# CircleRadon/TokenPacker

Hardware: NVIDIA H100
Metric: compressed_visual_tokens_per_sec (higher is better)
Workload: dtype bf16

## Files before the change

### tokenpacker_b200/csrc/tp_api.cu

```cuda
#include <limits.h>
#include <atomic>
#include <math.h>
#include <stdio.h>
#include <stdlib.h>
#include <string.h>
#include <map>
#include <tuple>
#include <vector>

#include "../../include/tokenpacker_b200.h"
#include "../../include/tokenpacker_b200_clip_tower.h"
#include "../../include/tokenpacker_b200_clip_tower_f16.h"
#include "../../include/tokenpacker_b200_clip_tower_train.h"
#include "../../include/tokenpacker_b200_clip_tower_ckpt.h"
#include "../../include/tokenpacker_b200_clip_tower_embed.h"
#include "../../include/tokenpacker_b200_clip_u8.h"
#include "../../include/tokenpacker_b200_hd_u8.h"
#include "../../include/tokenpacker_b200_input_grad.h"
#include "../../include/tokenpacker_b200_layers.h"
#include "../../include/tokenpacker_b200_jpeg.h"
#include "tp_gemm.cuh"
#include "tp_kernels.cuh"
#include "tp_backward.cuh"
#include "tp_clip_tower.cuh"
// ... 205 lines not shown
template <int kBlockN, bool kTower, bool kF16 = false>
int launch_gemm_tt(const GemmItem& it, const CUtensorMap& map_a, const CUtensorMap& map_b, int sms, cudaStream_t stream) {
  using Cfg = GemmConfig<kBlockN>;
  {
    static thread_local unsigned attr_done = 0;
    int dev = 0;
    TP_CUDA(cudaGetDevice(&dev));
    if (dev >= 32 || !(attr_done & (1u << dev))) {
      TP_CUDA(cudaFuncSetAttribute(tp_gemm_kernel<kBlockN, kTower, kF16>, cudaFuncAttributeMaxDynamicSharedMemorySize, Cfg::kSmemBytes));
      if (dev < 32) attr_done |= 1u << dev;
    }
  }
  const long long tiles = ((it.M + kBlockM - 1) / kBlockM) * ((it.N + kBlockN - 1) / kBlockN);
  const int grid = static_cast<int>(tiles < sms ? tiles : sms);
  GemmEpilogue ep = it.ep;
  TP_CUDA(launch_pdl(tp_gemm_kernel<kBlockN, kTower, kF16>, dim3(grid), dim3(kGemmThreads), Cfg::kSmemBytes, stream, map_a, map_b,
                     static_cast<int>(it.M), static_cast<int>(it.N), static_cast<int>(it.K), static_cast<int>(it.a.seg_rows), ep));
  return TP_OK;
}

template <int kBlockN>
int launch_gemm_t(const GemmItem& it, const CUtensorMap& map_a, const CUtensorMap& map_b, int sms, cudaStream_t stream) {
  switch (gemm_variant(it.ep)) {
    case 2: return launch_gemm_tt<kBlockN, true, true>(it, map_a, map_b, sms, stream);
    case 1: return launch_gemm_tt<kBlockN, true>(it, map_a, map_b, sms, stream);
    default: return launch_gemm_tt<kBlockN, false>(it, map_a, map_b, sms, stream);
  }
}

struct BuiltLaunch {
  GemmGroup g;
  PeerStores peers;
  int grid;
};

int build_pair_group(const GemmItem* items, int count, int sms, const FrontWork* front, BuiltLaunch* out) {
  using Cfg = Gemm2Config;
  GemmGroup& g = out->g;
  memset(&g, 0, sizeof(g));
  g.count = count;
  for (int i = 1; i < count; ++i)
    if (gemm_variant(items[i].ep) != gemm_variant(items[0].ep)) return TP_ERR_INVALID_ARGUMENT;
  if (count > 0 && gemm_variant(items[0].ep) != 0 && front != nullptr) return TP_ERR_INVALID_ARGUMENT;
  long long total = 0;
  for (int i = 0; i < count; ++i) {
    const GemmItem& it = items[i];
    GemmProblem& p = g.p[i];
    if (it.kind == 1) {
      if (it.N != kC || it.K != kC || it.a2 == nullptr || it.b2 == nullptr || (it.attn.s != 2 && it.attn.s != 4)) return TP_ERR_INVALID_ARGUMENT;
      TP_TRY(make_map_2d(&p.tmap_a, it.a.ptr, it.M, it.K, it.a.ld, kBlockM));
      TP_TRY(make_map_2d(&p.tmap_a2, it.a2, it.M, it.K, it.a.ld, kBlockM));
      TP_TRY(make_map_2d(&p.tmap_b, it.b, it.N, it.K, it.ldb, Cfg::kTileN / 2));
      TP_TRY(make_map_2d(&p.tmap_b2, it.b2, it.N, it.K, it.ldb, Cfg::kTileN / 2));
      p.kind = 1;
      p.attn = it.attn;
      p.a_parts = 1;
      p.M = static_cast<int>(it.M);
      p.N = static_cast<int>(it.N);
      p.K = static_cast<int>(it.K);
      p.num_n_blocks = 4;
      p.num_k_blocks = static_cast<int>(it.K / kBlockK);
      p.tiles_mn = static_cast<int>((it.M + Cfg::kTileM - 1) / Cfg::kTileM) * p.num_n_blocks;
      p.k_splits = 1;
      p.kb_per_split = p.num_k_blocks;
      p.num_tiles = p.tiles_mn;
      p.dep_counter = nullptr;
      total += p.num_tiles;
      continue;
    }
    if (it.tn == 1 && (it.b_parts > 1 || it.b_seg_rows != 0)) {
      if (it.b_parts < 1 || it.b_parts > kMaxAParts || it.N % (it.b_parts * Cfg::kTileN) != 0 || it.a.parts > 1 || it.a.seg_rows != 0 ||
          (it.b_seg_rows != 0 && (it.b_seg_rows % kBlockK != 0 || it.K % it.b_seg_rows != 0)))
        return TP_ERR_INVALID_ARGUMENT;
      TP_TRY(make_map_2d(&p.tmap_a, it.a.ptr, it.K, it.M, it.a.ld, 64));
      const long long np = it.N / it.b_parts;
      for (int q = 0; q < it.b_parts; ++q) {
// ... 51 lines not shown
        int rows = p.c_unit << lvl;
        if (rows > kBlockM || rows > it.ep.seg_len) rows = p.c_unit;
        TP_TRY(make_map_3d(lvl == 0 ? &p.tmap_c : &p.tmap_cx[lvl - 1], it.ep.c, it.M / it.ep.seg_len, it.ep.seg_len, it.N, it.ep.ldc,
                           it.ep.seg_stride * it.ep.ldc, rows));
      }
    } else {
      TP_TRY(make_map_2d(&p.tmap_c, it.ep.c, it.M, it.N, it.ep.ldc, kBlockM));
    }
    if (it.ep.dual) {
      if (!p.use_tma_store || c_segmented || it.ep.wm_s != 0 || it.n_peers > 0 || !it.ep.gelu || it.c_pre == nullptr || it.k_splits > 1)
        return TP_ERR_INVALID_ARGUMENT;
      TP_TRY(make_map_2d(&p.tmap_cx[0], it.c_pre, it.M, it.N, it.ld_pre, kBlockM));
    }
    p.M = static_cast<int>(it.M);
    p.N = static_cast<int>(it.N);
    p.K = static_cast<int>(it.K);
    p.a_seg_rows = static_cast<int>(it.a.seg_rows);
    p.num_n_blocks = static_cast<int>((it.N + Cfg::kTileN - 1) / Cfg::kTileN);
    p.num_k_blocks = static_cast<int>((it.K + kBlockK - 1) / kBlockK);
    p.tiles_mn = static_cast<int>((it.M + Cfg::kTileM - 1) / Cfg::kTileM) * p.num_n_blocks;
    p.k_splits = it.k_splits;
    p.kb_per_split = (p.num_k_blocks + p.k_splits - 1) / p.k_splits;
    if (static_cast<long long>(p.k_splits - 1) * p.kb_per_split >= p.num_k_blocks) return TP_ERR_INVALID_ARGUMENT;
    p.c_split_stride = it.M * it.ep.ldc;
    p.num_tiles = p.tiles_mn * p.k_splits;
    p.ep = it.ep;
    p.done_counter = it.done_counter;
    p.dep_counter = it.dep_counter;
    p.dep_target = it.dep_target;
    p.dep_shift = it.dep_shift;
    p.dep_span = it.dep_span;
    p.dep_src_blocks = it.dep_src_blocks;
    p.dep_per = it.dep_per;
    if ((p.done_counter != nullptr && !p.use_tma_store) || (p.dep_counter != nullptr && (it.tn || it.a.seg_rows != 0)))
      return TP_ERR_INVALID_ARGUMENT;
    p.peer_out = it.n_peers > 0 ? 1 : 0;
    total += p.num_tiles;
  }
  if (total > 0x7fffffffll) return TP_ERR_INVALID_ARGUMENT;
  g.total_tiles = static_cast<int>(total);
  if (front != nullptr) g.front = *front;
  PeerStores& peers = out->peers;
  memset(&peers, 0, sizeof(peers));
  int peer_item = -1;
  for (int i = 0; i < count; ++i)
    if (items[i].n_peers > 0 || g.p[i].c_seg_len != 0) {
      if (peer_item >= 0 && items[i].n_peers == 0 && items[peer_item].n_peers == 0 && g.p[i].c_seg_len > kBlockM) continue;
      if (peer_item >= 0) return TP_ERR_INVALID_ARGUMENT;
      peer_item = i;
    }
  if (peer_item >= 0) {
    const GemmItem& it0 = items[peer_item];
    const GemmProblem& p0 = g.p[peer_item];
    void* const local_dst[1] = {it0.ep.c};
    void* const* dst = it0.n_peers > 0 ? it0.peer_c : local_dst;
    const int n_dst = it0.n_peers > 0 ? it0.n_peers : 1;
    if (n_dst > kMaxPeers || it0.ep.seg_row_offset != nullptr) return TP_ERR_INVALID_ARGUMENT;
    const bool whole = p0.c_seg_len != 0 && p0.c_seg_len <= kBlockM;
    if (p0.c_seg_len != 0) {
      int worst = 0;
      for (int a0 = 0; a0 > -p0.c_seg_len; a0 -= p0.c_unit) {
        int pieces = 0, a = a0;
        while (a < kBlockM) {
          if (whole && a >= 0 && a + p0.c_seg_len <= kBlockM) {
            int k = 1;
            while (k < kWholeLevels && a + (k + 1) * p0.c_seg_len <= kBlockM) ++k;
            ++pieces;
// ... 11 lines not shown
    }
    for (int p = 0; p < n_dst; ++p) {
      if (p0.c_seg_len != 0) {
        const long long n_segs = it0.M / it0.ep.seg_len;
        for (int lvl = 0; lvl < kBoxLevels; ++lvl) {
          int rows = p0.c_unit << lvl;
          if (rows > kBlockM || rows > it0.ep.seg_len) rows = p0.c_unit;
          TP_TRY(make_map_3d(&peers.m[p][lvl], dst[p], n_segs, it0.ep.seg_len, it0.N, it0.ep.ldc, it0.ep.seg_stride * it0.ep.ldc, rows));
        }
        for (int k = 1; k <= kWholeLevels; ++k) {
          const int kk = (whole && k * it0.ep.seg_len <= kBlockM && k <= n_segs) ? k : 1;
          if (whole)
            TP_TRY(make_map_3d(&peers.m[p][kBoxLevels + k - 1], dst[p], n_segs, it0.ep.seg_len, it0.N, it0.ep.ldc,
                               it0.ep.seg_stride * it0.ep.ldc, it0.ep.seg_len, kk));
          else
            peers.m[p][kBoxLevels + k - 1] = peers.m[p][0];
        }
      } else {
        TP_TRY(make_map_2d(&peers.m[p][0], dst[p], it0.M, it0.N, it0.ep.ldc, kBlockM));
      }
    }
    peers.count = n_dst;
    peers.whole = whole ? 1 : 0;
    g.p[peer_item].peer_out = 1;
  }
  const long long max_pairs = sms / 2;
  const int grid = 2 * static_cast<int>(total < max_pairs ? total : max_pairs);
  for (int i = 0; i < count; ++i)
    if (g.p[i].dep_shift == 31) g.p[i].dep_target = grid;
  out->grid = grid;
  return TP_OK;
}

template <bool kTower, bool kF16 = false>
int launch_built_t(const BuiltLaunch& b, cudaStream_t stream) {
  using Cfg = Gemm2Config;
  {
    static thread_local unsigned attr_done = 0;
    int dev = 0;
    TP_CUDA(cudaGetDevice(&dev));
    if (dev >= 32 || !(attr_done & (1u << dev))) {
      TP_CUDA(cudaFuncSetAttribute(tp_gemm2_kernel<kTower, kF16>, cudaFuncAttributeMaxDynamicSharedMemorySize, Cfg::kSmemBytes));
      if (dev < 32) attr_done |= 1u << dev;
    }
  }
  TP_CUDA(launch_pdl(tp_gemm2_kernel<kTower, kF16>, dim3(b.grid), dim3(kGemmThreads), Cfg::kSmemBytes, stream, b.g, b.peers));
  return TP_OK;
}

int launch_built(const BuiltLaunch& b, cudaStream_t stream) {
  int variant = 0;
  for (int i = 0; i < b.g.count; ++i) variant = gemm_variant(b.g.p[i].ep) > variant ? gemm_variant(b.g.p[i].ep) : variant;
  switch (variant) {
    case 2: return launch_built_t<true, true>(b, stream);
    case 1: return launch_built_t<true>(b, stream);
    default: return launch_built_t<false>(b, stream);
  }
}

int launch_gemm_pair_group(const GemmItem* items, int count, int sms, cudaStream_t stream, const FrontWork* front = nullptr,
                           BuiltLaunch* built = nullptr) {
  BuiltLaunch local;
  BuiltLaunch* b = built != nullptr ? built : &local;
  TP_TRY(build_pair_group(items, count, sms, front, b));
  return launch_built(*b, stream);
}

int choose_kernel(const GemmItem& it, int count, int sms, int mode) {
  const bool c_segmented = it.ep.seg_row_offset == nullptr && !it.ep.out_f32 && it.ep.seg_stride != 0 && it.ep.seg_stride != it.ep.seg_len;
  const bool pair_ok = (it.N % 256 == 0) && sms >= 2 && !(c_segmented && seg_store_unit(it.ep.seg_len) < 4);
  const bool pair_only = it.n_peers > 0 || it.tn || it.ep.dual || it.a.parts > 1 || it.k_splits > 1 || it.ep.out_f32 || it.kind == 1 || it.ep.wm_s != 0;
  if (pair_only && !pair_ok) return -1;
  const bool needs_256 = it.ep.stats_out != nullptr;
  const long long kb = (it.K + kBlockK - 1) / kBlockK;
  auto waves = [](long long tiles, long long units) { return (tiles + units - 1) / units; };
  const long long t_pair = ((it.M + 255) / 256) * ((it.N + 255) / 256);
  const long long t_256 = ((it.M + 127) / 128) * ((it.N + 255) / 256);
  const long long t_128 = ((it.M + 127) / 128) * ((it.N + 127) / 128);
  const long long c_pair = pair_ok ? waves(t_pair, sms / 2) * kb * 1024 * 9 / 8 : LLONG_MAX;
  const long long c_256 = (it.N % 256 == 0) ? waves(t_256, sms) * kb * 1024 : LLONG_MAX;
  const long long c_128 = needs_256 ? LLONG_MAX : waves(t_128, sms) * kb * 512 * 6 / 5;
  const long long launch = 10000;
  const long long l_pair = pair_ok ? c_pair + launch / count : LLONG_MAX;
  const long long l_256 = c_256 == LLONG_MAX ? LLONG_MAX : c_256 + launch;
  const long long l_128 = c_128 == LLONG_MAX ? LLONG_MAX : c_128 + launch;
  int choice;
  if (pair_only || mode == 2 || mode == 3) choice = 0;
  else if (mode == 1) choice = (it.N % 256 == 0) ? 1 : 2;
  else if (l_pair <= l_256 && l_pair <= l_128) choice = 0;
  else choice = (l_256 <= l_128) ? 1 : 2;
  if (choice == 0 && !pair_ok) choice = (it.N % 256 == 0) ? 1 : 2;
  return choice;
}

int gemm_mode() {
  const char* mode_env = getenv("TP_GEMM_MODE");
  return mode_env != nullptr ? atoi(mode_env) : 0;
}

int launch_gemms(const GemmItem* items, int count, int sms, cudaStream_t stream) {
  if (count <= 0 || count > kMaxGroup || mixed_precision(items, count)) return TP_ERR_INVALID_ARGUMENT;
  const int mode = gemm_mode();
  int choice[kMaxGroup];
  CUtensorMap map_a[kMaxGroup], map_b[kMaxGroup];
  GemmItem grouped[kMaxGroup];
  int n_grouped = 0;
  BuiltLaunch pair;
  for (int i = 0; i < count; ++i) {
    TP_TRY(check_item(items[i]));
    const GemmItem& it = items[i];
    if (it.n_peers > 0 && count != 1) return TP_ERR_INVALID_ARGUMENT;
    choice[i] = choose_kernel(it, count, sms, mode);
    if (choice[i] < 0) return TP_ERR_INVALID_ARGUMENT;
    if (choice[i] == 0) {
      if (mode == 3) TP_TRY(build_pair_group(&it, 1, sms, nullptr, &pair));
      else grouped[n_grouped++] = it;
    } else {
      TP_TRY(make_one_cta_maps(it, choice[i] == 1 ? 256 : 128, &map_a[i], &map_b[i]));
    }
  }
  if (n_grouped > 0) TP_TRY(build_pair_group(grouped, n_grouped, sms, nullptr, &pair));
  for (int i = 0; i < count; ++i) {
    if (choice[i] == 0) {
      if (mode == 3) TP_TRY(launch_gemm_pair_group(&items[i], 1, sms, stream));
    } else if (choice[i] == 1) {
      TP_TRY(launch_gemm_t<256>(items[i], map_a[i], map_b[i], sms, stream));
    } else {
      TP_TRY(launch_gemm_t<128>(items[i], map_a[i], map_b[i], sms, stream));
    }
  }
  if (n_grouped > 0) TP_TRY(launch_built(pair, stream));
  return TP_OK;
}

int launch_front_s(int s, const __nv_bfloat16* x0, long long x0_stride, __nv_bfloat16* q, long long Q, cudaStream_t stream);

bool chain_enabled(int mode) {
  const char* e = getenv("TP_CHAIN");
  const bool chain_off = e != nullptr && atoi(e) == 0;
  return !chain_off && (mode == 0 || mode == 2);
}

bool chain_feasible(const GemmItem* items, int count, int sms, bool by_cost = true) {
  const int mode = gemm_mode();
  if (!chain_enabled(mode) || count <= 0 || count > kMaxGroup || sms < 2) return false;
  for (int i = 0; i < count; ++i) {
    if (check_item(items[i]) != TP_OK || items[i].ep.seg_row_offset != nullptr || items[i].N % 256 != 0) return false;
    if (by_cost && choose_kernel(items[i], count, sms, mode) != 0) return false;
  }
  return true;
}

int launch_chain(GemmItem* items, int count, int* flags, long long flag_capacity, const FrontWork* front, int sms, cudaStream_t stream,
                 BuiltLaunch* built = nullptr) {
  if (count <= 0 || count > kMaxGroup || mixed_precision(items, count)) return TP_ERR_INVALID_ARGUMENT;
  for (int i = 0; i < count; ++i) {
    const int deps[3] = {items[i].dep, items[i].dep2, items[i].dep3};
    for (int d : deps) {
      if (d == kDepFront ? front == nullptr : (d >= 0 && (d >= i || items[d].stage >= items[i].stage))) return TP_ERR_INVALID_ARGUMENT;
      if (d >= 0 && items[i].kind == 0 && items[d].kind == 0 && (items[d].M != items[i].M || items[i].a.seg_rows != 0)) return TP_ERR_INVALID_ARGUMENT;
    }
  }
  bool fused_items = false;
  for (int i = 0; i < count; ++i) fused_items = fused_items || items[i].kind == 1 || items[i].ep.wm_s != 0;
  const bool chain = flags != nullptr && chain_feasible(items, count, sms, !fused_items);
  if (chain) {
    long long used = 0;
    FrontWork fw;
    memset(&fw, 0, sizeof(fw));
    if (front != nullptr) {
      if (used + 1 > flag_capacity) return TP_ERR_WORKSPACE_TOO_SMALL;
      fw = *front;
      fw.done_counter = flags + used;
      used += 1;
    }
    for (int i = 0; i < count; ++i) {
      bool produces = false;
      for (int j = 0; j < count; ++j) produces = produces || items[j].dep == i || items[j].dep2 == i || items[j].dep3 == i;
      if (!produces) continue;
      const long long out_rows = items[i].kind == 1 ? items[i].M / (items[i].attn.s * items[i].attn.s) : items[i].M;
      const long long blocks = (out_rows + 255) / 256;
      if (used + blocks > flag_capacity) return TP_ERR_WORKSPACE_TOO_SMALL;
      items[i].done_counter = flags + used;
      if (items[i].kind == 1) {
        items[i].attn.done_counter = items[i].done_counter;
        items[i].done_counter = nullptr;
      }
      used += blocks;
    }
    auto counter_of = [&](int d) { return items[d].kind == 1 ? items[d].attn.done_counter : items[d].done_counter; };
    auto gemm_target = [&](int d) { return 4 * static_cast<int>((items[d].N + 255) / 256); };
    for (int i = 0; i < count; ++i) {
      GemmItem& it = items[i];
      if (it.kind == 1) {
        if (it.dep < 0 || it.dep2 < 0 || it.dep3 < 0 || items[it.dep].M != it.M || items[it.dep2].M != it.M) return TP_ERR_INVALID_ARGUMENT;
        it.attn.k_counter = counter_of(it.dep);
        it.attn.v_counter = counter_of(it.dep2);
        it.attn.kv_target = gemm_target(it.dep);
        it.attn.q_counter = counter_of(it.dep3);
        it.attn.q_target = gemm_target(it.dep3);
        continue;
      }
      const int d = it.dep;
      if (d == kDepFront) {
        it.dep_counter = fw.done_counter;
        it.dep_shift = 31;
      } else if (d >= 0 && items[d].kind == 1) {
        it.dep_counter = counter_of(d);
        it.dep_span = items[d].attn.s * items[d].attn.s;
        it.dep_src_blocks = static_cast<int>((items[d].M + 255) / 256);
        it.dep_per = 8;
      } else if (d >= 0) {
        it.dep_counter = counter_of(d);
        it.dep_target = gemm_target(d);
      }
    }
    return launch_gemm_pair_group(items, count, sms, stream, front != nullptr ? &fw : nullptr, built);
  }
  for (int i = 0; i < count; ++i)
    if (items[i].kind == 1 || items[i].ep.wm_s != 0) return TP_ERR_INVALID_ARGUMENT;
  if (front != nullptr) TP_TRY(launch_front_s(front->s, front->x0, front->crop_stride, front->q, front->n_queries, stream));
  for (int first = 0; first < count;) {
    int last = first;
    while (last + 1 < count && items[last + 1].stage == items[first].stage) ++last;
    TP_TRY(launch_gemms(items + first, last - first + 1, sms, stream));
    first = last + 1;
  }
  return TP_OK;
}

int launch_gemm(const AOperand& a, const void* b, long long ldb, long long M, long long N, long long K, const GemmEpilogue& ep,
                int sms, cudaStream_t stream) {
  const GemmItem it{a, b, ldb, M, N, K, ep};
  return launch_gemms(&it, 1, sms, stream);
}

GemmEpilogue plain_epilogue(void* c, long long ldc, const float* bias, int gelu) {
  GemmEpilogue ep;
  memset(&ep, 0, sizeof(ep));
  ep.c = static_cast<__nv_bfloat16*>(c);
  ep.ldc = ldc;
  ep.col_b = bias;
  ep.gelu = gelu;
  ep.alpha = 1.0f;
  ep.ln_inv_dim = 1.0f / kC;
  ep.ln_eps = 1e-6f;
  return ep;
}

struct PackedLayout {
  size_t w_kv0, b_kv0;
  size_t w_k2, b_k2, w_v2, b_v2;
  size_t w_ik, wsum_k, c_k;
  size_t w_iv, wsum_v, c_v;
  size_t w_q;
  size_t w_iq, wsum_q, c_q;
  size_t w_ot;
  size_t w_om, b_om;
  size_t w_m2, b_m2;
  size_t w_o, b_o, w_m0, b_m0;
  size_t total;
};

PackedLayout packed_layout(int H) {
  PackedLayout L;
  size_t off = 0;
  auto take = [&](size_t bytes) { size_t o = off; off = align_up(off + bytes, 256); return o; };
// ... 356 lines not shown
    g[5].attn.cst_v = wf(L.c_v);
    g[5].attn.s = s;
    g[5].attn.stats_slots = kStatSlots;
    g[5].attn.ln_inv_dim = 1.0f / kC;
    g[5].attn.ln_eps = 1e-6f;
    g[5].stage = 3;
    g[5].dep = 1;
    g[5].dep2 = 2;
    g[5].dep3 = 4;
    g[6] = GemmItem{AOperand{bf(W.ctx), kC, 0, 0}, P + L.w_om, kC, Q, H, kC, plain_epilogue(bf(W.h_m), H, wf(L.b_om), 1)};
    g[6].stage = 4;
    g[6].dep = 5;
    GemmEpilogue ep = plain_epilogue(out, H, wf(L.b_m2), 0);
    if (out_crop_rows != 0 && out_crop_rows != Mq) {
      if (out_crop_rows < Mq || out_crop_rows > 0x7fffffffll / H) return TP_ERR_INVALID_ARGUMENT;
      ep.seg_len = Mq;
      ep.seg_stride = static_cast<int>(out_crop_rows);
    }
    g[7] = GemmItem{AOperand{bf(W.h_m), H, 0, 0}, P + L.w_m2, H, Q, H, H, ep};
    g[7].peer_c = peer_out;
    g[7].n_peers = n_peers;
    g[7].stage = 5;
    g[7].dep = 6;
    FwdKey key;
    memset(&key, 0, sizeof(key));
    key.packed = packed; key.x0 = f.x0; key.out = out; key.ws = workspace;
    for (int i = 0; i < 4; ++i) key.xm[i] = f.xm[i];
    for (int i = 0; i < n_peers && i < kMaxPeers; ++i) key.peers[i] = peer_out[i];
    key.n = n_crops; key.s0 = f.x0_crop_stride; key.sm = f.xm_crop_stride; key.crop_rows = out_crop_rows;
    key.s = s; key.H = H; key.n_peers = n_peers; key.sms = dev.sms; key.parts = f.parts;
    if (chain_feasible(g, 8, dev.sms, false)) {
      for (FwdPlan& fp : g_fwd_plans)
        if (fp.valid && memcmp(&fp.key, &key, sizeof(key)) == 0) {
          TP_CUDA(launch_pdl(tp_gemm2_kernel<false>, dim3(fp.launch.grid), dim3(kGemmThreads), Gemm2Config::kSmemBytes, stream, fp.launch.g, fp.launch.peers));
          return TP_OK;
        }
      FwdPlan& slot = g_fwd_plans[g_fwd_next];
      g_fwd_next = (g_fwd_next + 1) % 4;
      slot.valid = false;
      TP_TRY(launch_chain(g, 8, flags, W.n_flags, &front, dev.sms, stream, &slot.launch));
      slot.key = key;
      slot.valid = true;
      return TP_OK;
    }
  }
  {
    GemmItem g[7];
    stage12_items(g, f, P, L, nullptr, bufs, R, Q);
    stage3_items(g + 4, P, L, bufs, R, Q);
    g[1].stage = g[2].stage = g[3].stage = 1;
    g[1].dep = g[2].dep = 0;
    g[3].dep = kDepFront;
    g[4].stage = g[5].stage = g[6].stage = 2;
    g[4].dep = 1;
    g[5].dep = 2;
    g[6].dep = 3;
    TP_TRY(launch_chain(g, 7, flags, flags_a + (Q + 255) / 256 + 1, &front, dev.sms, stream));
  }
  TP_TRY(launch_attn_s(s, bufs.q_p, bufs.k_p, bufs.v_p, bf(W.ctx), Q, stream));
  {
    GemmItem g[2];
    g[0] = GemmItem{AOperand{bf(W.ctx), kC, 0, 0}, P + L.w_om, kC, Q, H, kC, plain_epilogue(bf(W.h_m), H, wf(L.b_om), 1)};
    g[0].stage = 0;
    GemmEpilogue ep = plain_epilogue(out, H, wf(L.b_m2), 0);
    if (seg_row_offset != nullptr) {
      ep.seg_row_offset = reinterpret_cast<const long long*>(seg_row_offset);
      ep.seg_len = Mq;
    } else if (out_crop_rows != 0 && out_crop_rows != Mq) {
      if (out_crop_rows < Mq || out_crop_rows > 0x7fffffffll / H) return TP_ERR_INVALID_ARGUMENT;
      ep.seg_len = Mq;
      ep.seg_stride = static_cast<int>(out_crop_rows);
    }
    g[1] = GemmItem{AOperand{bf(W.h_m), H, 0, 0}, P + L.w_m2, H, Q, H, H, ep};
// ... 157 lines not shown
  TP_CUDA(e3);
  return TP_OK;
}

int tp_gemm_tn_bf16(const void* a, int64_t lda, const void* b, int64_t ldb, void* c, int64_t ldc, int64_t m, int64_t n, int64_t k,
                    float alpha, void* stream) {
  if (a == nullptr || b == nullptr || c == nullptr) return TP_ERR_INVALID_ARGUMENT;
  DeviceInfo dev;
  TP_TRY(device_info(&dev));
  GemmItem it{AOperand{a, lda, 0, 0}, b, ldb, m, n, k, plain_epilogue(c, ldc, nullptr, 0)};
  it.ep.alpha = alpha;
  it.tn = 1;
  return launch_gemms(&it, 1, dev.sms, static_cast<cudaStream_t>(stream));
}

int tp_gemm_nn_bf16(const void* a, int64_t lda, const void* b, int64_t ldb, void* c, int64_t ldc, int64_t m, int64_t n, int64_t k,
                    float alpha, void* stream) {
  if (a == nullptr || b == nullptr || c == nullptr) return TP_ERR_INVALID_ARGUMENT;
  DeviceInfo dev;
  TP_TRY(device_info(&dev));
  GemmItem it{AOperand{a, lda, 0, 0}, b, ldb, m, n, k, plain_epilogue(c, ldc, nullptr, 0)};
  it.ep.alpha = alpha;
  it.tn = 2;
  return launch_gemms(&it, 1, dev.sms, static_cast<cudaStream_t>(stream));
}

int tp_gemm_bf16(const void* a, int64_t lda, const void* b, int64_t ldb, void* c, int64_t ldc, int64_t m, int64_t n, int64_t k,
                 const float* bias, int gelu, float alpha, void* stream) {
  if (a == nullptr || b == nullptr || c == nullptr) return TP_ERR_INVALID_ARGUMENT;
  DeviceInfo dev;
  TP_TRY(device_info(&dev));
  GemmEpilogue ep = plain_epilogue(c, ldc, bias, gelu != 0 ? 1 : 0);
  ep.alpha = alpha;
  return launch_gemm(AOperand{a, lda, 0, 0}, b, ldb, m, n, k, ep, dev.sms, static_cast<cudaStream_t>(stream));
}

#include "tp_train.inl"

namespace {
struct GridPair { int h, w; };
const GridPair kGrid9[] = {{1,1},{1,2},{2,1},{1,3},{3,1},{2,2},{1,4},{4,1},{1,5},{5,1},{1,6},{6,1},{2,3},{3,2},{1,7},{7,1},
                           {4,2},{2,4},{1,8},{8,1},{3,3},{1,9},{9,1}};
const GridPair kGrid16x[] = {{2,5},{5,2},{2,6},{6,2},{3,4},{4,3},{2,7},{7,2},{3,5},{5,3},{2,8},{8,2},{4,4}};
const GridPair kGrid25x[] = {{3,6},{6,3},{2,9},{9,2},{4,5},{5,4},{2,10},{10,2},{3,7},{7,3},{11,2},{2,11},{4,6},{6,4},{12,2},{2,12},
                             {3,8},{8,3},{4,6},{6,4},{5,5}};

int grid_table(int patch_num, GridPair* out) {
  int n = 0;
  for (const GridPair& p : kGrid9) out[n++] = p;
  if (patch_num == 9) return n;
  for (const GridPair& p : kGrid16x) out[n++] = p;
  if (patch_num == 16) return n;
  for (const GridPair& p : kGrid25x) out[n++] = p;
  return n;
}

long long py_round(double v) { return static_cast<long long>(nearbyint(v)); }
}

int tp_hd_grid(int64_t h, int64_t w, int patch_num, int image_size, int* h_block, int* w_block) {
  if (h_block == nullptr || w_block == nullptr || h <= 0 || w <= 0 || image_size <= 0) return TP_ERR_INVALID_ARGUMENT;
  if (patch_num != 9 && patch_num != 16 && patch_num != 25) return TP_ERR_BAD_PATCH_NUM;
  GridPair table[64];
  const int n = grid_table(patch_num, table);
  const float fh = static_cast<float>(h), fw = static_cast<float>(w);
  volatile float bh = fh * 1.4f, bw = fw * 1.4f;
  volatile float area2 = bh * bw;
// ... 388 lines not shown
```

### tokenpacker_b200/csrc/tp_gemm.cuh

```cuda
#pragma once

#include "tp_ptx.cuh"

namespace tp {

struct GemmEpilogue {
  void* c;
  long long ldc;
  const float* col_a;
  const float* col_b;
  const float* stats_in;
  float* stats_out;
  const long long* seg_row_offset;
  int seg_len;
  int seg_stride;
  int stats_in_slots;
  int stats_out_slots;
  float ln_inv_dim;
  float ln_eps;
  float alpha;
  int gelu;
  int wm_s;
  int out_f32;
  int dual;
// ... 127 lines not shown
constexpr int kSlabRowBytes = kSlabCols * 2;
constexpr int kChunksPerSlab = kSlabCols / 32;
constexpr int kOutSlabBytes = 128 * kSlabRowBytes;

constexpr int kColPad = 4;
template <int kTileN>
__host__ __device__ constexpr int col_slot(int vec, int c) { return vec * (kTileN + 2 * kColPad) + c + (c >= kTileN / 2 ? kColPad : 0); }

__device__ __forceinline__ long long window_major_row(long long row, int s) {
  const long long n = row / 576;
  const int t = static_cast<int>(row - n * 576);
  const int tr = t / 24, tc = t - tr * 24;
  const int hb = tr / s, hi = tr - hb * s, wb = tc / s, wi = tc - wb * s;
  return n * 576 + ((hb * (24 / s) + wb) * s + hi) * s + wi;
}

__device__ __forceinline__ void ln_row_stats(const float* stats, long long row, int slots, float inv_dim, float eps, float& mu, float& rstd) {
  const float2* st = reinterpret_cast<const float2*>(stats) + row * slots;
  float t1 = 0.f, m2 = 0.f;
  for (int i = 0; i < slots; ++i) t1 = __fadd_rn(t1, st[i].x);
  const float inv_slots = rcp_rn_normal(static_cast<float>(slots));
  mu = __fmul_rn(t1, inv_slots);
  float between = 0.f;
  for (int i = 0; i < slots; ++i) {
    const float2 v = st[i];
    const float d = __fsub_rn(v.x, mu);
    between = fmaf(d, d, between);
    m2 = __fadd_rn(m2, v.y);
  }
  const float var = __fmul_rn(fmaf(between, __fmul_rn(inv_slots, rcp_rn_normal(inv_dim)), m2), inv_dim);
  rstd = rsqrtf(__fadd_rn(var, eps));
}

template <int kTileN, bool kTower = false, bool kF16 = false, int kSubPairs = 8>
__device__ __forceinline__ void epilogue_tile(const GemmEpilogue& ep, int M, int N, const float (&acc)[2][kTileN / 4], uint32_t scratch,
                                              int row, int rloc, int col_tile0, int half, const float* s_col, const OutStage& out,
                                              long long c_extra = 0) {
  constexpr int kColsPerHalf = kTileN / 2;
  constexpr int kChunks = kColsPerHalf / 32;
  const bool ln_fold = !kTower && ep.col_a != nullptr;
  const bool row_ok = row < M;
  float mu = 0.f, rstd = 1.f;
  if (ln_fold && row_ok) ln_row_stats(ep.stats_in, row, ep.stats_in_slots, ep.ln_inv_dim, ep.ln_eps, mu, rstd);
  long long dst_row = row;
  if (ep.seg_row_offset != nullptr && row_ok) {
    const int seg = row / ep.seg_len;
    dst_row = ep.seg_row_offset[seg] + (row - seg * ep.seg_len);
  } else if (ep.seg_stride != 0 && row_ok) {
    const int seg = row / ep.seg_len;
    dst_row = static_cast<long long>(seg) * ep.seg_stride + (row - seg * ep.seg_len);
  }
  __nv_bfloat16* c_row = static_cast<__nv_bfloat16*>(ep.c) + dst_row * ep.ldc;
  float* c_row32 = reinterpret_cast<float*>(ep.c) + c_extra + dst_row * ep.ldc;
  const uint32_t sa_addr = smem_u32(s_col + col_slot<kTileN>(0, half * kColsPerHalf));
  const uint32_t sb_addr = smem_u32(s_col + col_slot<kTileN>(1, half * kColsPerHalf));
  const uint32_t out_addr = out.buf != nullptr ? smem_u32(out.buf) : 0u;

  float s1 = 0.f, s2 = 0.f, shift = 0.f;
  const bool do_stats = !kTower && ep.stats_out != nullptr;
  const bool scale = ep.alpha != 1.0f;
  const uint64_t rstd2 = pk2(rstd), nmu2 = pk2(-mu), alpha2 = pk2(ep.alpha);
  uint32_t r[32];
#pragma unroll
  for (int chunk = 0; chunk < kChunks; ++chunk) {
    acc_chunk(acc, chunk, scratch, r);
    const int col0 = col_tile0 + half * kColsPerHalf + chunk * 32;
    const bool dual = !kTower && ep.dual != 0 && out.buf != nullptr;
    const uint32_t slab_pre = out.slab_seq + 2u * static_cast<uint32_t>(chunk / kChunksPerSlab);
    const uint32_t slab_q = dual ? slab_pre + 1u : out.slab_seq + static_cast<uint32_t>(chunk / kChunksPerSlab);
    const uint32_t slab_buf = slab_q & 1u;
    if (out.buf != nullptr && (chunk % kChunksPerSlab) == 0) {
      if (dual) mbar_wait(&out.empty_bar[slab_pre & 1u], ((slab_pre >> 1) & 1u) ^ 1u);
      mbar_wait(&out.empty_bar[slab_buf], ((slab_q >> 1) & 1u) ^ 1u);
    }
    if (col0 < N) {
#pragma unroll
      for (int sub = 0; sub < 16 / kSubPairs; ++sub) {
        const int lc = chunk * 32 + sub * kSubPairs * 2;
        uint64_t v[kSubPairs];
#pragma unroll
        for (int j = 0; j < kSubPairs; ++j)
          v[j] = pk2(__uint_as_float(r[sub * kSubPairs * 2 + 2 * j]), __uint_as_float(r[sub * kSubPairs * 2 + 2 * j + 1]));
        const uint32_t sb4 = sb_addr + static_cast<uint32_t>(lc) * 4u;
// ... 313 lines not shown
              tma_load_3d(sa + h * (Cfg::kABytes / 2), &tmap_a, &full_bar[stage], kb * kBlockK, g - seg * a_seg_rows, seg);
            }
          }
          tma_load_2d(sb, &tmap_b, &full_bar[stage], kb * kBlockK, n_blk * kBlockN);
          if (++stage == kStages) { stage = 0; phase ^= 1u; }
        }
      }
    }
    __syncwarp();
  } else {
    setmaxnreg_inc<kMmaRegs>();
    const int e = warp_idx - kEpiWarp0;
    const int half = e >> 2;
    const int rloc = epi_row_1cta(warp_idx & 3, lane);
    const int epi_tid = e * 32 + static_cast<int>(lane);
    const uint32_t scratch = smem_u32(s_scratch + e * kScratchBytesPerWarp);
    constexpr int kN = kBlockN / 2;
    int stage = 0;
    uint32_t phase = 0;
    float acc[2][kN / 2];
    for (int tile = blockIdx.x; tile < num_tiles; tile += gridDim.x) {
      const int m_blk = tile / num_n_blocks;
      const int n_blk = tile - m_blk * num_n_blocks;
      stage_col_vectors<kBlockN>(ep, N, n_blk * kBlockN, s_col, epi_tid, true);
      mma_tile<kN, 2, 0, 0, kF16>(acc, smem, Cfg::kStageBytes, 0, Cfg::kABytes + half * kN * kBlockK * 2, full_bar, empty_bar, kStages, stage,
                                  phase, num_k_blocks);
      const OutStage no_stage{nullptr, nullptr, nullptr, 0u};
      epilogue_tile<kBlockN, kTower, kF16>(ep, M, N, acc, scratch, m_blk * kBlockM + rloc, rloc, n_blk * kBlockN, half, s_col,
                                           no_stage);
    }
  }
}

struct Gemm2Config {
  static constexpr int kTileM = 256;
  static constexpr int kTileN = 256;
  static constexpr int kStages = 3;
  static constexpr int kOutBufs = 2;
  static constexpr int kABytes = kBlockM * kBlockK * 2;
  static constexpr int kBBytes = kTileN * kBlockK * 2;
  static constexpr int kStageBytes = kABytes + kBBytes;
  static constexpr int kOutBytes = 2 * kOutBufs * kOutSlabBytes;
  static constexpr int kColStageBytes = col_slot<kTileN>(2, 0) * 4;
  static constexpr int kBarrierBytes = (2 * kStages + 4 * kOutBufs) * 8;
  static constexpr int kSmemBytes = kStages * kStageBytes + kOutBytes + kScratchBytes + kColStageBytes + kBarrierBytes;
  static_assert(kSmemBytes <= 232448, "shared memory budget of an sm_90 SM (227 KiB)");
};

constexpr int kMaxGroup = 8;

constexpr int kMaxAParts = 4;

struct GemmProblem {
  CUtensorMap tmap_a, tmap_b, tmap_c;
  CUtensorMap tmap_cx[kBoxLevels - 1];
  CUtensorMap tmap_a2, tmap_b2;
  int kind;
  int c_wm_s;
  AttnParams attn;
  CUtensorMap tmap_a_more[kMaxAParts - 1];
  int a_parts;
  int a_kblocks_per_part;
  int b_parts;
  int b_nblocks_per_part;
  int b_seg_rows;
  int M, N, K;
  int a_seg_rows;
  int ab_mn_major;
  int use_tma_store;
  int c_seg_len;
  int c_unit;
  int num_n_blocks;
  int num_tiles;
  int num_k_blocks;
  int k_splits;
  int kb_per_split;
  int tiles_mn;
// ... 24 lines not shown
  int total_tiles;
  FrontWork front;
};

static_assert(sizeof(GemmGroup) + sizeof(PeerStores) <= 32764, "tp_gemm2_kernel's parameter block exceeds the 32 KB limit");

struct TileRef {
  const GemmProblem* pr;
  int m_blk, n_blk;
  int kb0, kb1;
  int split;
};

__device__ __forceinline__ TileRef decode_tile(const GemmGroup& g, int tile) {
  int p = 0;
  while (p + 1 < g.count && tile >= g.p[p].num_tiles) {
    tile -= g.p[p].num_tiles;
    ++p;
  }
  TileRef t;
  t.pr = &g.p[p];
  t.split = 0;
  if (t.pr->k_splits > 1) {
    t.split = tile / t.pr->tiles_mn;
    tile -= t.split * t.pr->tiles_mn;
  }
  t.m_blk = tile / t.pr->num_n_blocks;
  t.n_blk = tile - t.m_blk * t.pr->num_n_blocks;
  t.kb0 = t.split * t.pr->kb_per_split;
  t.kb1 = t.kb0 + t.pr->kb_per_split < t.pr->num_k_blocks ? t.kb0 + t.pr->kb_per_split : t.pr->num_k_blocks;
  return t;
}

template <bool kTower = false, bool kF16 = false>
__global__ void __launch_bounds__(kGemmThreads, 1)
tp_gemm2_kernel(const __grid_constant__ GemmGroup grp, const __grid_constant__ PeerStores peers) {
  static_assert(kTower || !kF16, "f16 instantiations are the tower's");
  using Cfg = Gemm2Config;
  constexpr int kStages = Cfg::kStages;
  constexpr int kTileN = Cfg::kTileN;

  extern __shared__ __align__(1024) uint8_t smem_raw[];
  uint8_t* smem = smem_raw;
  uint8_t* s_out = smem + kStages * Cfg::kStageBytes;
  uint8_t* s_scratch = s_out + Cfg::kOutBytes;
  float* s_col_base = reinterpret_cast<float*>(s_scratch + kScratchBytes);
  uint64_t* full_bar = reinterpret_cast<uint64_t*>(s_scratch + kScratchBytes + Cfg::kColStageBytes);
  uint64_t* empty_bar = full_bar + kStages;
  uint64_t* slab_full_bar = empty_bar + kStages;
  uint64_t* slab_empty_bar = slab_full_bar + 2 * Cfg::kOutBufs;

  const int warp_idx = __shfl_sync(0xffffffffu, static_cast<int>(threadIdx.x >> 5), 0);
  const uint32_t lane = lane_id();
  const uint32_t cta_rank = blockIdx.x & 1u;
  const int num_tiles = grp.total_tiles;
  const int pair_idx = static_cast<int>(blockIdx.x >> 1);
  const int num_pairs = static_cast<int>(gridDim.x >> 1);

  if (warp_idx == kTmaWarp && lane == 0) {
    for (int i = 0; i < grp.count; ++i) {
      tma_prefetch_desc(&grp.p[i].tmap_a);
      for (int q = 1; q < grp.p[i].a_parts; ++q) tma_prefetch_desc(&grp.p[i].tmap_a_more[q - 1]);
      tma_prefetch_desc(&grp.p[i].tmap_b);
      if (grp.p[i].kind == 1) {
        tma_prefetch_desc(&grp.p[i].tmap_a2);
        tma_prefetch_desc(&grp.p[i].tmap_b2);
      }
      if (grp.p[i].use_tma_store) tma_prefetch_desc(&grp.p[i].tmap_c);
    }
    for (int i = 0; i < kStages; ++i) {
      mbar_init(&full_bar[i], 1);
      mbar_init(&empty_bar[i], kNumEpiWarps);
    }
    for (int i = 0; i < 2 * Cfg::kOutBufs; ++i) {
      mbar_init(&slab_full_bar[i], kNumEpiWarps);
      mbar_init(&slab_empty_bar[i], 1);
    }
    fence_barrier_init();
  }
  __syncthreads();
  grid_dependency_wait();
  grid_launch_dependents();
  if (warp_idx < kNumEpiWarps) {
    setmaxnreg_inc<kMmaRegs>();
    const int e = warp_idx - kEpiWarp0;
    const int wg = e >> 2;
    const int rloc = epi_row(wg, warp_idx & 3, lane);
    const int half = epi_half(lane);
    const int epi_tid = e * 32 + static_cast<int>(lane);
    const uint32_t scratch = smem_u32(s_scratch + e * kScratchBytesPerWarp);
    int stage = 0;
    uint32_t phase = 0;
    uint32_t slab_seq = 0;
    float acc[2][kTileN / 4];
    if (!kTower && grp.front.x0 != nullptr) {
      const FrontWork& fw = grp.front;
      const int g = 24 / fw.s, mq = g * g;
      const int lo = (fw.s & 1) ? (fw.s - 1) / 2 : fw.s / 2 - 1;
      const long long items = fw.n_queries * 128;
      for (long long idx = static_cast<long long>(blockIdx.x) * kEpiThreads + epi_tid; idx < items; idx += static_cast<long long>(gridDim.x) * kEpiThreads) {
        const long long query = idx >> 7;
        const int vec = static_cast<int>(idx & 127);
        const long long n = query / mq;
        const int m = static_cast<int>(query - n * mq);
        const int hb = m / g, wb = m - hb * g;
        const __nv_bfloat16* base = fw.x0 + n * fw.crop_stride + vec * 8 + static_cast<long long>((hb * fw.s + lo) * 24 + wb * fw.s + lo) * 1024;
        uint4 o = __ldg(reinterpret_cast<const uint4*>(base));
// ... 23 lines not shown
      const int row_tile0 = t.m_blk * Cfg::kTileM + static_cast<int>(cta_rank) * kBlockM;
      const int row = row_tile0 + rloc;
      if (!kTower && pr.kind == 1) {
        const AttnParams& at = pr.attn;
        const int head = t.n_blk * 2 + half;
        GemmEpilogue vec;
        vec.col_a = at.wsum_k;
        vec.col_b = at.cst_k;
        stage_col_vectors<kTileN>(vec, pr.N, t.n_blk * kTileN, s_col, epi_tid, true);
        mma_tile<kTileN, 1, 0, 0>(acc, smem, Cfg::kStageBytes, wg * 8192, Cfg::kABytes, full_bar, empty_bar, kStages, stage, phase, pr.num_k_blocks);
        const float p = attn_scores(at, pr.M, acc, scratch, row, head, half, s_col);
        vec.col_a = at.wsum_v;
        vec.col_b = at.cst_v;
        stage_col_vectors<kTileN>(vec, pr.N, t.n_blk * kTileN, s_col, epi_tid, true);
        mma_tile<kTileN, 1, 0, 0>(acc, smem, Cfg::kStageBytes, wg * 8192, Cfg::kABytes, full_bar, empty_bar, kStages, stage, phase, pr.num_k_blocks);
        attn_pv(at, pr.M, acc, scratch, row, head, half, p, s_col);
        if (at.done_counter != nullptr) {
          named_bar_sync(kEpiBarrierId, kEpiThreads);
          if (epi_tid == 0) {
            __threadfence();
            red_release_gpu_add(at.done_counter + ((static_cast<long long>(t.m_blk) * Cfg::kTileM / (at.s * at.s)) >> 8), 1);
          }
        }
        continue;
      }
      stage_col_vectors<kTileN>(pr.ep, pr.N, t.n_blk * kTileN, s_col, epi_tid, true);
      const int n_kb = t.kb1 - t.kb0;
      if (!kTower && pr.ab_mn_major == 1)
        mma_tile<kTileN, 1, 1, 1>(acc, smem, Cfg::kStageBytes, wg * 8192, Cfg::kABytes, full_bar, empty_bar, kStages, stage, phase, n_kb);
      else if (!kTower && pr.ab_mn_major == 2)
        mma_tile<kTileN, 1, 0, 1>(acc, smem, Cfg::kStageBytes, wg * 8192, Cfg::kABytes, full_bar, empty_bar, kStages, stage, phase, n_kb);
      else
        mma_tile<kTileN, 1, 0, 0, kF16>(acc, smem, Cfg::kStageBytes, wg * 8192, Cfg::kABytes, full_bar, empty_bar, kStages, stage, phase, n_kb);
      const OutStage out{pr.use_tma_store ? s_out + half * Cfg::kOutBufs * kOutSlabBytes : nullptr, slab_full_bar + half * Cfg::kOutBufs,
                         slab_empty_bar + half * Cfg::kOutBufs, slab_seq};
      if (pr.use_tma_store) slab_seq += (kTileN / 2 / kSlabCols) * (pr.ep.dual ? 2 : 1);
      epilogue_tile<kTileN, kTower, kF16, 4>(pr.ep, pr.M, pr.N, acc, scratch, row, rloc, t.n_blk * kTileN, half, s_col, out,
                                    static_cast<long long>(t.split) * pr.c_split_stride);
    }
  } else {
    setmaxnreg_dec<kAuxRegs>();
  if (warp_idx == kTmaWarp) {
    int stage = 0;
    uint32_t phase = 0;
    for (int tile = pair_idx; tile < num_tiles; tile += num_pairs) {
      const TileRef t = decode_tile(grp, tile);
      const GemmProblem& pr = *t.pr;
      const int row0 = t.m_blk * Cfg::kTileM + static_cast<int>(cta_rank) * kBlockM;
      const int brow0 = t.n_blk * kTileN;
      if (pr.dep_counter != nullptr) {
        int target = pr.dep_target;
        if (pr.dep_span != 0) {
          const int lo = t.m_blk * pr.dep_span;
          const int hi = lo + pr.dep_span < pr.dep_src_blocks ? lo + pr.dep_span : pr.dep_src_blocks;
          target = (hi - lo) * pr.dep_per;
        }
        wait_counter_at_least(pr.dep_counter + (t.m_blk >> pr.dep_shift), target);
        fence_proxy_async_all();
      }
      if (pr.kind == 1) {
        const AttnParams& at = pr.attn;
        if (at.k_counter != nullptr) {
          const long long r_lo = static_cast<long long>(t.m_blk) * Cfg::kTileM;
          const long long r_hi = r_lo + Cfg::kTileM < pr.M ? r_lo + Cfg::kTileM : pr.M;
          const int n_blocks = (pr.M + Cfg::kTileM - 1) / Cfg::kTileM;
          int b_lo = static_cast<int>((r_lo / 576) * 576 / Cfg::kTileM);
          int b_hi = static_cast<int>((((r_hi - 1) / 576 + 1) * 576 + Cfg::kTileM - 1) / Cfg::kTileM);
          if (b_hi > n_blocks) b_hi = n_blocks;
          for (int b = b_lo; b < b_hi; ++b) {
            wait_counter_at_least(at.k_counter + b, at.kv_target);
            wait_counter_at_least(at.v_counter + b, at.kv_target);
// ... 44 lines not shown
            } else {
              tma_load_3d(sa, ta, &full_bar[stage], ka, srow0, seg0);
              tma_load_3d(sa + Cfg::kABytes / 2, ta, &full_bar[stage], ka, srow1, seg1);
            }
          }
          if (pr.ab_mn_major == 0) {
            tma_load_2d(sb, &pr.tmap_b, &full_bar[stage], kb * kBlockK, brow0);
            tma_load_2d(sb + Cfg::kBBytes / 2, &pr.tmap_b, &full_bar[stage], kb * kBlockK, brow0 + kTileN / 2);
          } else if (pr.b_parts <= 1 && pr.b_seg_rows == 0) {
#pragma unroll
            for (int a4 = 0; a4 < 4; ++a4)
              tma_load_2d(sb + a4 * (Cfg::kBBytes / 4), &pr.tmap_b, &full_bar[stage], brow0 + a4 * 64, kb * kBlockK);
          } else {
            const int bpart = pr.b_parts > 1 ? t.n_blk / pr.b_nblocks_per_part : 0;
            const CUtensorMap* tb = bpart == 0 ? &pr.tmap_b : &pr.tmap_a_more[bpart - 1];
            const int bcol0 = bpart == 0 ? brow0 : (t.n_blk - bpart * pr.b_nblocks_per_part) * kTileN;
            if (pr.b_seg_rows == 0) {
#pragma unroll
              for (int a4 = 0; a4 < 4; ++a4)
                tma_load_2d(sb + a4 * (Cfg::kBBytes / 4), tb, &full_bar[stage], bcol0 + a4 * 64, kb * kBlockK);
            } else {
              const int g = kb * kBlockK;
              const int seg = g / pr.b_seg_rows;
#pragma unroll
              for (int a4 = 0; a4 < 4; ++a4)
                tma_load_3d(sb + a4 * (Cfg::kBBytes / 4), tb, &full_bar[stage], bcol0 + a4 * 64, g - seg * pr.b_seg_rows, seg);
            }
          }
        }
        __syncwarp();
        if (++stage == kStages) { stage = 0; phase ^= 1u; }
      }
    }
  } else if (warp_idx == kStoreWarp0 || warp_idx == kStoreWarp0 + 1) {
    const int half = warp_idx - kStoreWarp0;
    uint64_t* full = slab_full_bar + half * Cfg::kOutBufs;
    uint64_t* empty = slab_empty_bar + half * Cfg::kOutBufs;
    uint32_t q = 0;
    for (int tile = pair_idx; tile < num_tiles; tile += num_pairs) {
      const TileRef t = decode_tile(grp, tile);
      const GemmProblem& pr = *t.pr;
      if (!pr.use_tma_store) continue;
      const int row_tile0 = t.m_blk * Cfg::kTileM + static_cast<int>(cta_rank) * kBlockM;
      const bool to_peers = pr.peer_out != 0 && peers.count > 0;
      const int n_maps = to_peers ? peers.count : 1;
      const int dual = pr.ep.dual != 0 ? 1 : 0;
      for (int slab = 0; slab < (kTileN / 2 / kSlabCols) << dual; ++slab, ++q) {
        const uint32_t buf = q & 1u;
        mbar_wait(&full[buf], (q >> 1) & 1u);
        {
          const uint8_t* src = s_out + (half * Cfg::kOutBufs + static_cast<int>(buf)) * kOutSlabBytes;
          const int col = t.n_blk * kTileN + half * (kTileN / 2) + (slab >> dual) * kSlabCols;
          constexpr int kJobsPerLane = 3;
          const CUtensorMap* jmap[kJobsPerLane];
          int jlo[kJobsPerLane], jc1[kJobsPerLane], jc2[kJobsPerLane], jc3[kJobsPerLane], jc4[kJobsPerLane];
#pragma unroll
          for (int k = 0; k < kJobsPerLane; ++k) jmap[k] = nullptr;
          int job = 0;
          auto add = [&](const CUtensorMap* mp, int lo, int c1, int c2, int c3, int c4) {
#pragma unroll
            for (int k = 0; k < kJobsPerLane; ++k)
              if (job == static_cast<int>(lane) + 32 * k) { jmap[k] = mp; jlo[k] = lo; jc1[k] = c1; jc2[k] = c2; jc3[k] = c3; jc4[k] = c4; }
            ++job;
          };
          int kind = 2;
          if (pr.c_wm_s != 0) {
            kind = 5;
// ... 75 lines not shown
```

Before: 3.719 million.

## Add slab-free GEMM variant storing directly from registers with deeper pipeline

Adds a kSlabs template switch to the paired GEMM kernel. When off, the epilogue writes results straight from registers to global memory, handling window-major rows directly. This removes the shared-memory output slabs, their barriers and the TMA store warps. The freed shared memory pays for a fourth load stage, and a done-counter release replaces the store-warp signalling. The forward chain plan and the plain gemm API opt into this path, trading TMA-store coalescing for deeper load pipelining and less epilogue synchronisation.

After: 3.827 million (median of 6 runs). 1.03x the previous value.

```diff
diff --git a/tokenpacker_b200/csrc/tp_api.cu b/tokenpacker_b200/csrc/tp_api.cu
--- a/tokenpacker_b200/csrc/tp_api.cu
+++ b/tokenpacker_b200/csrc/tp_api.cu
@@ -261,16 +261,26 @@
   GemmGroup g;
   PeerStores peers;
   int grid;
+  int slabs;
 };
 
-int build_pair_group(const GemmItem* items, int count, int sms, const FrontWork* front, BuiltLaunch* out) {
-  using Cfg = Gemm2Config;
+int g_force_slabs = -1;
+
+int build_pair_group(const GemmItem* items, int count, int sms, const FrontWork* front, BuiltLaunch* out, bool reg_store = false) {
+  using Cfg = Gemm2Config<>;
   GemmGroup& g = out->g;
   memset(&g, 0, sizeof(g));
   g.count = count;
   for (int i = 1; i < count; ++i)
     if (gemm_variant(items[i].ep) != gemm_variant(items[0].ep)) return TP_ERR_INVALID_ARGUMENT;
   if (count > 0 && gemm_variant(items[0].ep) != 0 && front != nullptr) return TP_ERR_INVALID_ARGUMENT;
+  bool slabs = !(g_force_slabs == 0 || (g_force_slabs < 0 && reg_store));
+  for (int i = 0; i < count; ++i) {
+    const GemmEpilogue& ep = items[i].ep;
+    const bool c_segmented = ep.seg_row_offset == nullptr && !ep.out_f32 && ep.seg_stride != 0 && ep.seg_stride != ep.seg_len;
+    slabs = slabs || items[i].n_peers > 0 || c_segmented || ep.dual || gemm_variant(ep) != 0;
+  }
+  out->slabs = slabs ? 1 : 0;
   long long total = 0;
   for (int i = 0; i < count; ++i) {
     const GemmItem& it = items[i];
@@ -388,7 +398,7 @@
     p.dep_span = it.dep_span;
     p.dep_src_blocks = it.dep_src_blocks;
     p.dep_per = it.dep_per;
-    if ((p.done_counter != nullptr && !p.use_tma_store) || (p.dep_counter != nullptr && (it.tn || it.a.seg_rows != 0)))
+    if ((slabs && p.done_counter != nullptr && !p.use_tma_store) || (p.dep_counter != nullptr && (it.tn || it.a.seg_rows != 0)))
       return TP_ERR_INVALID_ARGUMENT;
     p.peer_out = it.n_peers > 0 ? 1 : 0;
     total += p.num_tiles;
@@ -466,19 +476,19 @@
   return TP_OK;
 }
 
-template <bool kTower, bool kF16 = false>
+template <bool kTower, bool kF16 = false, bool kSlabs = true>
 int launch_built_t(const BuiltLaunch& b, cudaStream_t stream) {
-  using Cfg = Gemm2Config;
+  using Cfg = Gemm2Config<kSlabs>;
   {
     static thread_local unsigned attr_done = 0;
     int dev = 0;
     TP_CUDA(cudaGetDevice(&dev));
     if (dev >= 32 || !(attr_done & (1u << dev))) {
-      TP_CUDA(cudaFuncSetAttribute(tp_gemm2_kernel<kTower, kF16>, cudaFuncAttributeMaxDynamicSharedMemorySize, Cfg::kSmemBytes));
+      TP_CUDA(cudaFuncSetAttribute(tp_gemm2_kernel<kTower, kF16, kSlabs>, cudaFuncAttributeMaxDynamicSharedMemorySize, Cfg::kSmemBytes));
       if (dev < 32) attr_done |= 1u << dev;
     }
   }
-  TP_CUDA(launch_pdl(tp_gemm2_kernel<kTower, kF16>, dim3(b.grid), dim3(kGemmThreads), Cfg::kSmemBytes, stream, b.g, b.peers));
+  TP_CUDA(launch_pdl(tp_gemm2_kernel<kTower, kF16, kSlabs>, dim3(b.grid), dim3(kGemmThreads), Cfg::kSmemBytes, stream, b.g, b.peers));
   return TP_OK;
 }
 
@@ -488,15 +498,15 @@
   switch (variant) {
     case 2: return launch_built_t<true, true>(b, stream);
     case 1: return launch_built_t<true>(b, stream);
-    default: return launch_built_t<false>(b, stream);
+    default: return b.slabs ? launch_built_t<false>(b, stream) : launch_built_t<false, false, false>(b, stream);
   }
 }
 
 int launch_gemm_pair_group(const GemmItem* items, int count, int sms, cudaStream_t stream, const FrontWork* front = nullptr,
-                           BuiltLaunch* built = nullptr) {
+                           BuiltLaunch* built = nullptr, bool reg_store = false) {
   BuiltLaunch local;
   BuiltLaunch* b = built != nullptr ? built : &local;
-  TP_TRY(build_pair_group(items, count, sms, front, b));
+  TP_TRY(build_pair_group(items, count, sms, front, b, reg_store));
   return launch_built(*b, stream);
 }
 
@@ -532,7 +542,7 @@
   return mode_env != nullptr ? atoi(mode_env) : 0;
 }
 
-int launch_gemms(const GemmItem* items, int count, int sms, cudaStream_t stream) {
+int launch_gemms(const GemmItem* items, int count, int sms, cudaStream_t stream, bool reg_store = false) {
   if (count <= 0 || count > kMaxGroup || mixed_precision(items, count)) return TP_ERR_INVALID_ARGUMENT;
   const int mode = gemm_mode();
   int choice[kMaxGroup];
@@ -547,16 +557,16 @@
     choice[i] = choose_kernel(it, count, sms, mode);
     if (choice[i] < 0) return TP_ERR_INVALID_ARGUMENT;
     if (choice[i] == 0) {
-      if (mode == 3) TP_TRY(build_pair_group(&it, 1, sms, nullptr, &pair));
+      if (mode == 3) TP_TRY(build_pair_group(&it, 1, sms, nullptr, &pair, reg_store));
       else grouped[n_grouped++] = it;
     } else {
       TP_TRY(make_one_cta_maps(it, choice[i] == 1 ? 256 : 128, &map_a[i], &map_b[i]));
     }
   }
-  if (n_grouped > 0) TP_TRY(build_pair_group(grouped, n_grouped, sms, nullptr, &pair));
+  if (n_grouped > 0) TP_TRY(build_pair_group(grouped, n_grouped, sms, nullptr, &pair, reg_store));
   for (int i = 0; i < count; ++i) {
     if (choice[i] == 0) {
-      if (mode == 3) TP_TRY(launch_gemm_pair_group(&items[i], 1, sms, stream));
+      if (mode == 3) TP_TRY(launch_gemm_pair_group(&items[i], 1, sms, stream, nullptr, nullptr, reg_store));
     } else if (choice[i] == 1) {
       TP_TRY(launch_gemm_t<256>(items[i], map_a[i], map_b[i], sms, stream));
     } else {
@@ -586,7 +596,7 @@
 }
 
 int launch_chain(GemmItem* items, int count, int* flags, long long flag_capacity, const FrontWork* front, int sms, cudaStream_t stream,
-                 BuiltLaunch* built = nullptr) {
+                 BuiltLaunch* built = nullptr, bool reg_store = false) {
   if (count <= 0 || count > kMaxGroup || mixed_precision(items, count)) return TP_ERR_INVALID_ARGUMENT;
   for (int i = 0; i < count; ++i) {
     const int deps[3] = {items[i].dep, items[i].dep2, items[i].dep3};
@@ -649,7 +659,7 @@
         it.dep_target = gemm_target(d);
       }
     }
-    return launch_gemm_pair_group(items, count, sms, stream, front != nullptr ? &fw : nullptr, built);
+    return launch_gemm_pair_group(items, count, sms, stream, front != nullptr ? &fw : nullptr, built, reg_store);
   }
   for (int i = 0; i < count; ++i)
     if (items[i].kind == 1 || items[i].ep.wm_s != 0) return TP_ERR_INVALID_ARGUMENT;
@@ -657,16 +667,16 @@
   for (int first = 0; first < count;) {
     int last = first;
     while (last + 1 < count && items[last + 1].stage == items[first].stage) ++last;
-    TP_TRY(launch_gemms(items + first, last - first + 1, sms, stream));
+    TP_TRY(launch_gemms(items + first, last - first + 1, sms, stream, reg_store));
     first = last + 1;
   }
   return TP_OK;
 }
 
 int launch_gemm(const AOperand& a, const void* b, long long ldb, long long M, long long N, long long K, const GemmEpilogue& ep,
-                int sms, cudaStream_t stream) {
+                int sms, cudaStream_t stream, bool reg_store = false) {
   const GemmItem it{a, b, ldb, M, N, K, ep};
-  return launch_gemms(&it, 1, sms, stream);
+  return launch_gemms(&it, 1, sms, stream, reg_store);
 }
 
 GemmEpilogue plain_epilogue(void* c, long long ldc, const float* bias, int gelu) {
@@ -1089,13 +1099,12 @@
     if (chain_feasible(g, 8, dev.sms, false)) {
       for (FwdPlan& fp : g_fwd_plans)
         if (fp.valid && memcmp(&fp.key, &key, sizeof(key)) == 0) {
-          TP_CUDA(launch_pdl(tp_gemm2_kernel<false>, dim3(fp.launch.grid), dim3(kGemmThreads), Gemm2Config::kSmemBytes, stream, fp.launch.g, fp.launch.peers));
-          return TP_OK;
+          return launch_built(fp.launch, stream);
         }
       FwdPlan& slot = g_fwd_plans[g_fwd_next];
       g_fwd_next = (g_fwd_next + 1) % 4;
       slot.valid = false;
-      TP_TRY(launch_chain(g, 8, flags, W.n_flags, &front, dev.sms, stream, &slot.launch));
+      TP_TRY(launch_chain(g, 8, flags, W.n_flags, &front, dev.sms, stream, &slot.launch, true));
       slot.key = key;
       slot.valid = true;
       return TP_OK;
@@ -1319,7 +1328,7 @@
   TP_TRY(device_info(&dev));
   GemmEpilogue ep = plain_epilogue(c, ldc, bias, gelu != 0 ? 1 : 0);
   ep.alpha = alpha;
-  return launch_gemm(AOperand{a, lda, 0, 0}, b, ldb, m, n, k, ep, dev.sms, static_cast<cudaStream_t>(stream));
+  return launch_gemm(AOperand{a, lda, 0, 0}, b, ldb, m, n, k, ep, dev.sms, static_cast<cudaStream_t>(stream), true);
 }
 
 #include "tp_train.inl"
diff --git a/tokenpacker_b200/csrc/tp_gemm.cuh b/tokenpacker_b200/csrc/tp_gemm.cuh
--- a/tokenpacker_b200/csrc/tp_gemm.cuh
+++ b/tokenpacker_b200/csrc/tp_gemm.cuh
@@ -183,7 +183,7 @@
   rstd = rsqrtf(__fadd_rn(var, eps));
 }
 
-template <int kTileN, bool kTower = false, bool kF16 = false, int kSubPairs = 8>
+template <int kTileN, bool kTower = false, bool kF16 = false, int kSubPairs = 8, bool kDirectWm = false>
 __device__ __forceinline__ void epilogue_tile(const GemmEpilogue& ep, int M, int N, const float (&acc)[2][kTileN / 4], uint32_t scratch,
                                               int row, int rloc, int col_tile0, int half, const float* s_col, const OutStage& out,
                                               long long c_extra = 0) {
@@ -200,6 +200,8 @@
   } else if (ep.seg_stride != 0 && row_ok) {
     const int seg = row / ep.seg_len;
     dst_row = static_cast<long long>(seg) * ep.seg_stride + (row - seg * ep.seg_len);
+  } else if (kDirectWm && ep.wm_s != 0 && row_ok) {
+    dst_row = window_major_row(row, ep.wm_s);
   }
   __nv_bfloat16* c_row = static_cast<__nv_bfloat16*>(ep.c) + dst_row * ep.ldc;
   float* c_row32 = reinterpret_cast<float*>(ep.c) + c_extra + dst_row * ep.ldc;
@@ -579,17 +581,18 @@
   }
 }
 
+template <bool kSlabs = true>
 struct Gemm2Config {
   static constexpr int kTileM = 256;
   static constexpr int kTileN = 256;
-  static constexpr int kStages = 3;
+  static constexpr int kStages = kSlabs ? 3 : 4;
   static constexpr int kOutBufs = 2;
   static constexpr int kABytes = kBlockM * kBlockK * 2;
   static constexpr int kBBytes = kTileN * kBlockK * 2;
   static constexpr int kStageBytes = kABytes + kBBytes;
-  static constexpr int kOutBytes = 2 * kOutBufs * kOutSlabBytes;
+  static constexpr int kOutBytes = kSlabs ? 2 * kOutBufs * kOutSlabBytes : 0;
   static constexpr int kColStageBytes = col_slot<kTileN>(2, 0) * 4;
-  static constexpr int kBarrierBytes = (2 * kStages + 4 * kOutBufs) * 8;
+  static constexpr int kBarrierBytes = (2 * kStages + (kSlabs ? 4 * kOutBufs : 0)) * 8;
   static constexpr int kSmemBytes = kStages * kStageBytes + kOutBytes + kScratchBytes + kColStageBytes + kBarrierBytes;
   static_assert(kSmemBytes <= 232448, "shared memory budget of an sm_90 SM (227 KiB)");
 };
@@ -680,11 +683,12 @@
   return t;
 }
 
-template <bool kTower = false, bool kF16 = false>
+template <bool kTower = false, bool kF16 = false, bool kSlabs = true>
 __global__ void __launch_bounds__(kGemmThreads, 1)
 tp_gemm2_kernel(const __grid_constant__ GemmGroup grp, const __grid_constant__ PeerStores peers) {
   static_assert(kTower || !kF16, "f16 instantiations are the tower's");
-  using Cfg = Gemm2Config;
+  static_assert(kSlabs || !kTower, "the tower's launches keep the slab configuration");
+  using Cfg = Gemm2Config<kSlabs>;
   constexpr int kStages = Cfg::kStages;
   constexpr int kTileN = Cfg::kTileN;
 
@@ -714,13 +718,13 @@
         tma_prefetch_desc(&grp.p[i].tmap_a2);
         tma_prefetch_desc(&grp.p[i].tmap_b2);
       }
-      if (grp.p[i].use_tma_store) tma_prefetch_desc(&grp.p[i].tmap_c);
+      if (kSlabs && grp.p[i].use_tma_store) tma_prefetch_desc(&grp.p[i].tmap_c);
     }
     for (int i = 0; i < kStages; ++i) {
       mbar_init(&full_bar[i], 1);
       mbar_init(&empty_bar[i], kNumEpiWarps);
     }
-    for (int i = 0; i < 2 * Cfg::kOutBufs; ++i) {
+    for (int i = 0; i < (kSlabs ? 2 * Cfg::kOutBufs : 0); ++i) {
       mbar_init(&slab_full_bar[i], kNumEpiWarps);
       mbar_init(&slab_empty_bar[i], 1);
     }
@@ -810,11 +814,24 @@
         mma_tile<kTileN, 1, 0, 1>(acc, smem, Cfg::kStageBytes, wg * 8192, Cfg::kABytes, full_bar, empty_bar, kStages, stage, phase, n_kb);
       else
         mma_tile<kTileN, 1, 0, 0, kF16>(acc, smem, Cfg::kStageBytes, wg * 8192, Cfg::kABytes, full_bar, empty_bar, kStages, stage, phase, n_kb);
-      const OutStage out{pr.use_tma_store ? s_out + half * Cfg::kOutBufs * kOutSlabBytes : nullptr, slab_full_bar + half * Cfg::kOutBufs,
-                         slab_empty_bar + half * Cfg::kOutBufs, slab_seq};
-      if (pr.use_tma_store) slab_seq += (kTileN / 2 / kSlabCols) * (pr.ep.dual ? 2 : 1);
-      epilogue_tile<kTileN, kTower, kF16, 4>(pr.ep, pr.M, pr.N, acc, scratch, row, rloc, t.n_blk * kTileN, half, s_col, out,
-                                    static_cast<long long>(t.split) * pr.c_split_stride);
+      if constexpr (kSlabs) {
+        const OutStage out{pr.use_tma_store ? s_out + half * Cfg::kOutBufs * kOutSlabBytes : nullptr, slab_full_bar + half * Cfg::kOutBufs,
+                           slab_empty_bar + half * Cfg::kOutBufs, slab_seq};
+        if (pr.use_tma_store) slab_seq += (kTileN / 2 / kSlabCols) * (pr.ep.dual ? 2 : 1);
+        epilogue_tile<kTileN, kTower, kF16, 4>(pr.ep, pr.M, pr.N, acc, scratch, row, rloc, t.n_blk * kTileN, half, s_col, out,
+                                      static_cast<long long>(t.split) * pr.c_split_stride);
+      } else {
+        const OutStage no_stage{nullptr, nullptr, nullptr, 0u};
+        epilogue_tile<kTileN, kTower, kF16, 4, true>(pr.ep, pr.M, pr.N, acc, scratch, row, rloc, t.n_blk * kTileN, half, s_col, no_stage,
+                                                     static_cast<long long>(t.split) * pr.c_split_stride);
+        if (pr.done_counter != nullptr) {
+          named_bar_sync(kEpiBarrierId, kEpiThreads);
+          if (epi_tid == 0) {
+            __threadfence();
+            red_release_gpu_add(pr.done_counter + t.m_blk, 2);
+          }
+        }
+      }
     }
   } else {
     setmaxnreg_dec<kAuxRegs>();
@@ -925,7 +942,7 @@
         if (++stage == kStages) { stage = 0; phase ^= 1u; }
       }
     }
-  } else if (warp_idx == kStoreWarp0 || warp_idx == kStoreWarp0 + 1) {
+  } else if (kSlabs && (warp_idx == kStoreWarp0 || warp_idx == kStoreWarp0 + 1)) {
     const int half = warp_idx - kStoreWarp0;
     uint64_t* full = slab_full_bar + half * Cfg::kOutBufs;
     uint64_t* empty = slab_empty_bar + half * Cfg::kOutBufs;
```
